# alanross/AlvaAR

Measured on AMD Instinct MI355X. Metric: frames/sec @640x480 2000kp; local-BA residuals/sec (20KFx3k pts), higher is better.
Workload: dtype u8/i16 image stages, f32 KLT, f64 pose+BA; 1 GPU; configs[1]: 640x480 RGBA stream, ~2000 keypoints/frame (cell 12), System::findCameraPose dataflow (fb-KLT -> P3P-LMedS -> PnP; keyframes: detect + describe, triangulate, map matching, local BA) via alva_system_find_camera_pose_device, steady state, frames resident in HBM; parallelism=1 independent camera streams, one per GPU, no collective on the data path

## Files before the change

### alvaar_amd/csrc/ba.hip

```cpp
#include "common.hpp"
#include "lm_device.hpp"
#include "wave_utils.hpp"
#include <chrono>
#include <cstdlib>
#include <algorithm>
#include <cmath>
#include <numeric>

namespace {

typedef double double4_t __attribute__((ext_vector_type(4)));

struct BaDev {
    int nKf, nPt, nObs, inv, dp, nc, n6, NP;
    int npd;
    int kpad;
    double K[4], huber_a;
    const int *obsKf;
    const double *obsUv;
    const int *ptPtr;
    const int *ancKf;
    const double *ancUv;
    const int *cidx;
    double *rowcol;
    const int *kfOf;
    const int *pairPerm;
    const int *pairPtr;
    double *Jobs;
    double *rs;
    double *chi2;
    uint8_t *depth;
    double *ptCost;
    double *Hpp;
    double *gp;
    double *Wt;
    double *M;
    double *Hcc;
    double *gc;
    double *sc, *sp, *dc, *dpd;
    double *hinv;
    double *Zt;
    double *Gpart;
    double *S;
    double *yc;
    double *yp;
    double *scal;
    double *h_scal;
    long long seq;
    double *partial;
    unsigned long long *dbg;
};
#define SOLVE_STAMP(k) do { if (B.dbg && threadIdx.x == 0) B.dbg[3072 + (k)] = wall_clock64(); } while (0)
#define ASM_STAMP(k) do { if (B.dbg && threadIdx.x == 0) B.dbg[3072 + 48 + (k)] = wall_clock64(); } while (0)

constexpr int KSPLIT = 8;

__device__ __forceinline__ double wave_sum(double v) {
#pragma unroll
    for (int off = 32; off > 0; off >>= 1) v += __shfl_down(v, off);
    return __shfl(v, 0);
}

template<bool INV, bool WANT_J>
__device__ __forceinline__ void point_body(const BaDev &B, const double *__restrict__ poses, const double *__restrict__ pts, const int BX_, const int BY_) {
    const int lane = threadIdx.x & 63;
    const int p = BX_ * 4 + (threadIdx.x >> 6);
    if (p >= B.nPt) return;
    constexpr int DP = INV ? 1 : 3;
    const int o0 = B.ptPtr[p], o1 = B.ptPtr[p + 1];
    double X[3], dJl[3] = {0, 0, 0};
    int a = -1;
    if (INV) {
        a = B.ancKf[p];
        Se3 Ta;
        se3_from_pose7(poses + 7 * a, Ta);
        const double zanch = 1.0 / pts[p];
        const double ap[3] = {zanch * ((B.ancUv[2 * p] - B.K[2]) / B.K[0]), zanch * ((B.ancUv[2 * p + 1] - B.K[3]) / B.K[1]), zanch};
        double Ra[3];
        for (int i = 0; i < 3; i++) Ra[i] = Ta.R[3 * i] * ap[0] + Ta.R[3 * i + 1] * ap[1] + Ta.R[3 * i + 2] * ap[2];
        for (int i = 0; i < 3; i++) {
            X[i] = Ra[i] + Ta.t[i];
            dJl[i] = -zanch * Ra[i];
        }
    } else {
        for (int i = 0; i < 3; i++) X[i] = pts[3 * p + i];
    }
    double cost = 0, hpp[DP * DP], gpv[DP], wanc[6 * DP];
#pragma unroll
    for (int i = 0; i < DP * DP; i++) hpp[i] = 0;
#pragma unroll
    for (int i = 0; i < DP; i++) gpv[i] = 0;
#pragma unroll
    for (int i = 0; i < 6 * DP; i++) wanc[i] = 0;
    for (int o = o0 + lane; o < o1; o += 64) {
        const int k = B.obsKf[o];
        Se3 T;
        se3_from_pose7(poses + 7 * k, T);
        double r[2], JR[6], chi2;
        int dpz;
        reproj<WANT_J>(T, B.K, X, B.obsUv[2 * o], B.obsUv[2 * o + 1], r, JR, chi2, dpz);
        B.chi2[o] = chi2;
        B.depth[o] = (uint8_t) dpz;
        double rho0, rho1;
        huber_rho(chi2, B.huber_a, 1, rho0, rho1);
        cost += 0.5 * rho0;
        if (WANT_J) {
            const double s = sqrt(rho1);
            double JH[6], Jo[12], Je[2 * DP];
// ... 57 lines not shown
                    const double w = wave_sum(wanc[i]);
                    if (lane == 0) B.Wt[(size_t) p * B.NP + 6 * ca + i] = w;
                }
            }
        }
    }
}
template<bool INV, bool WANT_J>
__global__ void __launch_bounds__(256) k_point(BaDev B, const double *__restrict__ poses, const double *__restrict__ pts) {
    point_body<INV, WANT_J>(B, poses, pts, blockIdx.x, blockIdx.y);
}

__device__ __forceinline__ void pairs_body(const BaDev &B, const int BX_, const int BY_) {
    const int lane = threadIdx.x & 63, wave = threadIdx.x >> 6;
    const int key = BX_;
    __shared__ double s_part[4][28];
    double v[32];
#pragma unroll
    for (int i = 0; i < 32; i++) v[i] = 0;
    for (int q = B.pairPtr[key] + threadIdx.x; q < B.pairPtr[key + 1]; q += 256) {
        const int o = B.pairPerm[q];
        double J[12];
#pragma unroll
        for (int i = 0; i < 12; i++) J[i] = B.Jobs[(size_t) o * 12 + i];
        const double r0 = B.rs[2 * (size_t) o], r1 = B.rs[2 * (size_t) o + 1];
        int t = 0;
#pragma unroll
        for (int x = 0; x < 6; x++) {
            v[21 + x] += J[x] * r0 + J[6 + x] * r1;
#pragma unroll
            for (int y = x; y < 6; y++) v[t++] += J[x] * J[y] + J[6 + x] * J[6 + y];
        }
    }
    wave_reduce_scatter32(v);
    if (!(lane & 1) && (lane >> 1) < 27) s_part[wave][lane >> 1] = v[0];
    __syncthreads();
    if (threadIdx.x < 27) B.M[(size_t) key * 27 + threadIdx.x] = ((s_part[0][threadIdx.x] + s_part[1][threadIdx.x]) + s_part[2][threadIdx.x]) + s_part[3][threadIdx.x];
}
__global__ void __launch_bounds__(256) k_pairs(BaDev B) {
    pairs_body(B, blockIdx.x, blockIdx.y);
}

__device__ __forceinline__ int tri6(int x, int y) {
    if (x > y) {
        const int t = x;
        x = y;
        y = t;
    }
    return x * 6 - x * (x - 1) / 2 + (y - x);
}

constexpr int ASM_NT = 1024;
static inline size_t assemble_lds(int n_kf) { return (size_t) 2 * n_kf * 27 * sizeof(double); }
__device__ __forceinline__ void assemble_body(const BaDev &B, int first) {
    extern __shared__ double s_rc[];
    __shared__ double s_red[5][ASM_NT / 64];
    __shared__ int s_kfof[64];
    const int nKf = B.nKf, n6 = B.n6, tid = threadIdx.x;
    ASM_STAMP(0);
    if (tid < B.nc && tid < 64) s_kfof[tid] = B.kfOf[tid];
    double *rowsum = s_rc, *colsum = s_rc + (size_t) nKf * 27;
    for (int e = tid; e < 2 * nKf * 27; e += ASM_NT) {
        const bool col = e >= nKf * 27;
        const int q = col ? e - nKf * 27 : e, k = q / 27, t = q - 27 * k;
        const size_t stride = col ? (size_t) nKf * 27 : 27, first_e = col ? (size_t) k * 27 + t : (size_t) k * nKf * 27 + t;
        double acc = 0;
        for (int j0 = 0; j0 < nKf; j0 += 8) {
            double v[8];
#pragma unroll
            for (int u = 0; u < 8; u++) v[u] = j0 + u < nKf ? B.M[first_e + (size_t) (j0 + u) * stride] : 0.0;
#pragma unroll
            for (int u = 0; u < 8; u++)
                if (j0 + u < nKf) acc += v[u];
        }
        s_rc[e] = acc;
    }
    __syncthreads();
    ASM_STAMP(1);
    double gm = 0;
    {
        const double *__restrict__ M = B.M;
        const int lane = tid & 63, wave = tid >> 6, NW = ASM_NT / 64;
        const bool lds_map = B.nc <= 64;
        for (int r0 = wave; r0 < n6; r0 += 2 * NW) {
            for (int c0 = lane; c0 < n6; c0 += 128) {
                double v[4];
                int er[4], ec[4];
#pragma unroll
                for (int u = 0; u < 4; u++) {
                    const int r = r0 + (u >> 1) * NW, c = c0 + (u & 1) * 64;
                    er[u] = r; ec[u] = c;
                    v[u] = 0;
                    if (r < n6 && c < n6) {
                        const int cr = r / 6, cc = c / 6, x = r - 6 * cr, y = c - 6 * cc;
                        const int kr = lds_map ? s_kfof[cr] : B.kfOf[cr], kc = lds_map ? s_kfof[cc] : B.kfOf[cc];
                        const int t = tri6(x, y);
                        if (B.inv) {
                            if (kr == kc) v[u] = rowsum[kr * 27 + t] + colsum[kr * 27 + t];
                            else v[u] = -(M[(size_t) (kr * nKf + kc) * 27 + t] + M[(size_t) (kc * nKf + kr) * 27 + t]);
                        } else {
                            if (kr == kc) v[u] = M[(size_t) (kr * nKf + kr) * 27 + t];
                        }
                    }
                }
#pragma unroll
                for (int u = 0; u < 4; u++)
                    if (er[u] < n6 && ec[u] < n6) {
                        B.Hcc[(size_t) er[u] * n6 + ec[u]] = v[u];
                        if (first && er[u] == ec[u]) B.sc[er[u]] = 1.0 / (1.0 + sqrt(v[u]));
                    }
            }
        }
        for (int r = tid; r < n6; r += ASM_NT) {
            const int cr = r / 6, x = r - 6 * cr, kr = lds_map ? s_kfof[cr] : B.kfOf[cr];
            const double g = B.inv ? rowsum[kr * 27 + 21 + x] - colsum[kr * 27 + 21 + x] : M[(size_t) (kr * nKf + kr) * 27 + 21 + x];
            B.gc[r] = g;
            gm = fmax(gm, fabs(g));
        }
    }
    ASM_STAMP(2);
    if (first)
        for (int i = tid; i < B.npd; i += ASM_NT) {
            const int p = i / B.dp, x = i % B.dp;
            B.sp[i] = 1.0 / (1.0 + sqrt(B.Hpp[(size_t) p * B.dp * B.dp + x * B.dp + x]));
        }
    double cost = 0, mcc = 0, sn = 0, xn = 0;
    for (int i = tid; i < B.npd; i += ASM_NT) gm = fmax(gm, fabs(B.gp[i]));
    for (int p = tid; p < B.nPt; p += ASM_NT) {
        cost += B.ptCost[p];
        mcc += B.partial[3 * (size_t) p];
        sn += B.partial[3 * (size_t) p + 1];
        xn += B.partial[3 * (size_t) p + 2];
    }
    const int lane = tid & 63, wave = tid >> 6;
#pragma unroll
    for (int off = 32; off > 0; off >>= 1) {
        gm = fmax(gm, __shfl_xor(gm, off));
        cost += __shfl_xor(cost, off);
        mcc += __shfl_xor(mcc, off);
        sn += __shfl_xor(sn, off);
        xn += __shfl_xor(xn, off);
    }
    if (lane == 0) {
        s_red[0][wave] = gm; s_red[1][wave] = cost; s_red[2][wave] = mcc; s_red[3][wave] = sn; s_red[4][wave] = xn;
    }
    __syncthreads();
    ASM_STAMP(3);
    if (tid == 0) {
        double g2 = 0, c2 = 0, m2 = 0, s2 = 0, x2 = 0;
        for (int w = 0; w < ASM_NT / 64; w++) {
            g2 = fmax(g2, s_red[0][w]);
            c2 += s_red[1][w]; m2 += s_red[2][w]; s2 += s_red[3][w]; x2 += s_red[4][w];
        }
        const double *cam = B.partial + 3 * (size_t) B.nPt;
        B.scal[0] = c2;
        B.scal[3] = g2;
        B.scal[1] = m2 + cam[0];
        B.scal[2] = s2 + cam[1];
        B.scal[4] = x2 + cam[2];
        if (B.h_scal) {
            B.h_scal[0] = c2; B.h_scal[1] = m2 + cam[0]; B.h_scal[2] = s2 + cam[1]; B.h_scal[3] = g2;
            B.h_scal[4] = x2 + cam[2]; B.h_scal[5] = B.scal[5]; B.h_scal[6] = B.scal[6]; B.h_scal[7] = B.scal[7];
            __threadfence_system();
            __hip_atomic_store(reinterpret_cast<long long *>(B.h_scal + 8), B.seq, __ATOMIC_RELEASE, __HIP_MEMORY_SCOPE_SYSTEM);
        }
    }
}
__global__ void __launch_bounds__(ASM_NT) k_assemble(BaDev B, int first) { assemble_body(B, first); }

template<int DP>
__device__ __forceinline__ void prep_body(const BaDev &B, double radius, int refresh, const int BX_, const int BY_) {
    const int lane = threadIdx.x & 63;
    const int p = BX_ * 4 + (threadIdx.x >> 6);
    if (p >= B.nPt) return;
    double Mx[DP * DP], Hi[DP * DP], L[DP * DP], gs[DP], dpd[DP];
#pragma unroll
    for (int x = 0; x < DP; x++) {
        const int i = p * DP + x;
        if (refresh) {
            dpd[x] = fmin(fmax(B.Hpp[(size_t) p * DP * DP + x * DP + x] * B.sp[i] * B.sp[i], 1e-6), 1e32);
            if (lane == 0) B.dpd[i] = dpd[x];
        } else {
            dpd[x] = B.dpd[i];
        }
    }
#pragma unroll
    for (int x = 0; x < DP; x++) {
        gs[x] = B.gp[(size_t) p * DP + x] * B.sp[p * DP + x];
#pragma unroll
        for (int y = 0; y < DP; y++)
            Mx[x * DP + y] = B.Hpp[(size_t) p * DP * DP + x * DP + y] * B.sp[p * DP + x] * B.sp[p * DP + y] + (x == y ? dpd[x] / radius : 0.0);
    }
    if (DP == 1) {
        Hi[0] = 1.0 / Mx[0];
        L[0] = sqrt(Hi[0]);
    } else {
        for (int c = 0; c < DP; c++) {
            double A3[DP * DP], e[DP];
            for (int i = 0; i < DP * DP; i++) A3[i] = Mx[i];
            for (int i = 0; i < DP; i++) e[i] = (i == c);
            chol_solve_dense(A3, e, DP);
            for (int i = 0; i < DP; i++) Hi[i * DP + c] = e[i];
        }
        for (int i = 0; i < DP * DP; i++) L[i] = 0;
        for (int j = 0; j < DP; j++) {
            double d = Hi[j * DP + j];
            for (int k = 0; k < j; k++) d -= L[j * DP + k] * L[j * DP + k];
            d = sqrt(d);
            L[j * DP + j] = d;
            for (int i = j + 1; i < DP; i++) {
                double s = Hi[i * DP + j];
                for (int k = 0; k < j; k++) s -= L[i * DP + k] * L[j * DP + k];
                L[i * DP + j] = s / d;
            }
        }
    }
    if (lane == 0)
        for (int i = 0; i < DP * DP; i++) B.hinv[(size_t) p * DP * DP + i] = Hi[i];
    for (int r = lane; r < B.NP; r += 64) {
#pragma unroll
        for (int y = 0; y < DP; y++) {
            double v = 0;
            if (r < B.n6) {
#pragma unroll
                for (int x = 0; x < DP; x++) v += B.sc[r] * B.Wt[((size_t) p * DP + x) * B.NP + r] * B.sp[p * DP + x] * L[x * DP + y];
            } else if (r == B.n6) {
#pragma unroll
                for (int x = 0; x < DP; x++) v += L[x * DP + y] * gs[x];
            }
            B.Zt[((size_t) p * DP + y) * B.NP + r] = v;
        }
    }
}
template<int DP>
__global__ void __launch_bounds__(256) k_prep(BaDev B, double radius, int refresh) {
    prep_body<DP>(B, radius, refresh, blockIdx.x, blockIdx.y);
}

__device__ __forceinline__ void gemm_body(const BaDev &B, const int BX_, const int BY_) {
    const int tiles = B.NP / 16;
    const int ti = BX_ / tiles, tj = BX_ % tiles, ks = BY_;
    const int lane = threadIdx.x;
    const int chunk = B.kpad / KSPLIT;
    const int k0 = ks * chunk;
    double4_t acc = {0, 0, 0, 0};
    const double *Za = B.Zt + (size_t) (k0 + (lane >> 4)) * B.NP + ti * 16 + (lane & 15);
    const double *Zb = B.Zt + (size_t) (k0 + (lane >> 4)) * B.NP + tj * 16 + (lane & 15);
    int k = 0;
    for (; k + 32 <= chunk; k += 32) {
        double a[8], b[8];
#pragma unroll
        for (int u = 0; u < 8; u++) {
            a[u] = Za[(size_t) (k + 4 * u) * B.NP];
            b[u] = Zb[(size_t) (k + 4 * u) * B.NP];
        }
#pragma unroll
        for (int u = 0; u < 8; u++) acc = __builtin_amdgcn_mfma_f64_16x16x4f64(a[u], b[u], acc, 0, 0, 0);
    }
    for (; k < chunk; k += 4) {
        const double a = Za[(size_t) k * B.NP], b = Zb[(size_t) k * B.NP];
        acc = __builtin_amdgcn_mfma_f64_16x16x4f64(a, b, acc, 0, 0, 0);
    }
    double *G = B.Gpart + ((size_t) ks * B.NP + ti * 16) * B.NP + tj * 16;
#pragma unroll
    for (int r = 0; r < 4; r++) G[(size_t) ((lane >> 4) + 4 * r) * B.NP + (lane & 15)] = acc[r];
}
__global__ void __launch_bounds__(64) k_gemm(BaDev B) {
    gemm_body(B, blockIdx.x, blockIdx.y);
}

#ifndef ALVA_SOLVE_LOOKAHEAD
#define ALVA_SOLVE_LOOKAHEAD 1
#endif
constexpr int SOLVE_NT = 256, NB = 16;

__device__ __forceinline__ void reduced_system_body(const BaDev &B, double radius, int refresh, const int BX_, const int BY_) {
    const int n = B.n6, np = (n + NB - 1) / NB * NB, ld = np + 1;
    const int e = BX_ * 256 + threadIdx.x;
    if (e < np * np) {
        const int r = e / np, c = e - r * np;
        double v = r == c ? 1.0 : 0.0;
        if (r < n && c < n) {
            double g = 0;
#pragma unroll
            for (int ks = 0; ks < KSPLIT; ks++) g += B.Gpart[((size_t) ks * B.NP + r) * B.NP + c];
            const double h = B.Hcc[(size_t) r * n + c] * B.sc[r] * B.sc[c];
            v = h - g;
            if (r == c) {
                double dcr = B.dc[r];
                if (refresh) {
                    dcr = fmin(fmax(h, 1e-6), 1e32);
                    B.dc[r] = dcr;
                }
                v += dcr / radius;
            }
        }
        B.S[(size_t) r * ld + c] = v;
    } else if (e < np * np + np) {
        const int r = e - np * np;
        double v = 0;
        if (r < n) {
            double g = 0;
#pragma unroll
            for (int ks = 0; ks < KSPLIT; ks++) g += B.Gpart[((size_t) ks * B.NP + r) * B.NP + n];
            v = B.gc[r] * B.sc[r] - g;
        }
        B.S[(size_t) np * ld + r] = v;
    }
}
__global__ void __launch_bounds__(256) k_reduced_system(BaDev B, double radius, int refresh) {
    reduced_system_body(B, radius, refresh, blockIdx.x, blockIdx.y);
}

template<bool IN_LDS>
__device__ __forceinline__ void solve_body(const BaDev &B, double radius, const int BX_, const int BY_) {
    extern __shared__ double s_S[];
    const int n = B.n6, np = (n + NB - 1) / NB * NB, ld = np + 1, nb = np / NB;
    __shared__ double s_z[NB];
    __shared__ int s_ok;
    SOLVE_STAMP(0);
    double *S = IN_LDS ? s_S : B.S;
    double *y = IN_LDS ? s_S + (size_t) np * ld : B.S + (size_t) np * ld;
    constexpr int TILE_LUT = 1024;
    __shared__ unsigned short s_tile[TILE_LUT];
    auto fill_lut = [&]() {
        for (int t = threadIdx.x; t < TILE_LUT; t += SOLVE_NT) {
            int ta = (int) ((sqrtf(8.f * (float) t + 1.f) - 1.f) * 0.5f);
            while (ta * (ta + 1) / 2 > t) ta--;
            while ((ta + 1) * (ta + 2) / 2 <= t) ta++;
            s_tile[t] = (unsigned short) ((ta << 8) | (t - ta * (ta + 1) / 2));
        }
    };
    if (IN_LDS) {
        const int total = np * ld + np;
        bool lut_done = false;
        for (int e0 = threadIdx.x; e0 < total || !lut_done; e0 += 32 * SOLVE_NT) {
            double v[32];
#pragma unroll
            for (int u = 0; u < 32; u++) {
                const int e = e0 + u * SOLVE_NT;
                v[u] = e < total ? B.S[e] : 0.0;
            }
            if (!lut_done) {
                fill_lut();
                lut_done = true;
            }
#pragma unroll
            for (int u = 0; u < 32; u++) {
                const int e = e0 + u * SOLVE_NT;
                if (e < total) s_S[e] = v[u];
            }
        }
    } else {
        fill_lut();
    }
    if (threadIdx.x == 0) s_ok = 1;
    __syncthreads();
    SOLVE_STAMP(1);
    const int lane = threadIdx.x & 63;
    auto diag_factor = [&](const int base) {
// ... 441 lines not shown
        L.gmax = scal[3];
        L.last = L.cur;
    } else {
        const int cand = 1 - L.cur;
        L.last = cand;
        const double cand_cost = scal[0], mcc = scal[1], step_norm = sqrt(scal[2]);
        const bool okstep = scal[5] != 0.0 && isfinite(mcc);
        if (!okstep || !(mcc > 0)) {
            if (++L.invalid >= 5) {
                L.ok = 0;
                stop = true;
            } else {
                lm.rejected();
                L.nsummaries++;
            }
        } else {
            L.invalid = 0;
            if (step_norm <= 1e-8 * (L.x_norm + 1e-8)) stop = true;
            else if (fabs(L.x_cost - cand_cost) <= L.function_tolerance * L.x_cost) stop = true;
            else {
                const double rel = (L.x_cost - cand_cost) / mcc;
                if (rel > 1e-3) {
                    L.cur = cand;
                    L.x_cost = cand_cost;
                    L.gmax = scal[3];
                    L.x_norm = sqrt(scal[4]);
                    lm.accepted(rel);
                    L.nsucc++;
                } else {
                    lm.rejected();
                }
                L.nsummaries++;
            }
        }
    }
    L.radius = lm.radius; L.decrease_factor = lm.decrease_factor; L.reuse_diagonal = lm.reuse_diagonal;
    if (stop || L.iteration >= L.max_iters || L.gmax <= 1e-10 || L.radius <= 1e-32) {
        L.step = 0;
        return;
    }
    L.iteration++;
    L.diag = L.reuse_diagonal ? 0 : 1;
    L.reuse_diagonal = 1;
    L.step = 1;
}

#define LM_EVAL_SEL(first)                                  \
    if (!(first) && !L->step) return;                       \
    const int set = (first) ? L->cur : 1 - L->cur;          \
    const BaDev &B = dB[set];
template<bool INV>
__global__ void __launch_bounds__(256) k_point_lm(const BaDev *__restrict__ dB, const BaLmDev *__restrict__ L, int first) {
    LM_EVAL_SEL(first)
    point_body<INV, true>(B, L->P[set], L->T[set], blockIdx.x, 0);
}
__global__ void __launch_bounds__(256) k_pairs_lm(const BaDev *__restrict__ dB, const BaLmDev *__restrict__ L, int first) {
    LM_EVAL_SEL(first)
    pairs_body(B, blockIdx.x, 0);
}
__global__ void __launch_bounds__(ASM_NT) k_assemble_lm(const BaDev *__restrict__ dB, BaLmDev *L, int first) {
    LM_EVAL_SEL(first)
    assemble_body(B, first);
    if (threadIdx.x == 0) {
        BaLmDev S = *L;
        lm_after_eval(S, B.scal, first);
        S.evals++;
        *L = S;
        double *h = S.h_pub + ((S.evals & 1) ? 16 : 0);
        h[0] = S.step; h[1] = S.iteration; h[2] = S.nsummaries; h[3] = S.initial; h[4] = S.x_cost; h[5] = S.nsucc; h[6] = S.ok;
        h[7] = (double) (S.cur | (S.last << 8));
        __threadfence_system();
        __hip_atomic_store(reinterpret_cast<long long *>(S.h_pub + 8), S.evals, __ATOMIC_RELEASE, __HIP_MEMORY_SCOPE_SYSTEM);
    }
}
template<int DP>
__global__ void __launch_bounds__(256) k_prep_lm(const BaDev *__restrict__ dB, const BaLmDev *__restrict__ L) {
    if (!L->step) return;
    prep_body<DP>(dB[L->cur], L->radius, L->diag, blockIdx.x, 0);
}
__global__ void __launch_bounds__(64) k_gemm_lm(const BaDev *__restrict__ dB, const BaLmDev *__restrict__ L) {
    if (!L->step) return;
    gemm_body(dB[L->cur], blockIdx.x, blockIdx.y);
}
__global__ void __launch_bounds__(256) k_reduced_system_lm(const BaDev *__restrict__ dB, const BaLmDev *__restrict__ L) {
    if (!L->step) return;
    reduced_system_body(dB[L->cur], L->radius, L->diag, blockIdx.x, 0);
}
template<bool IN_LDS>
__global__ void __launch_bounds__(SOLVE_NT) k_solve_lm(const BaDev *__restrict__ dB, const BaLmDev *__restrict__ L) {
    if (!L->step) return;
    solve_body<IN_LDS>(dB[L->cur], L->radius, 0, 0);
}
template<int DP>
__global__ void __launch_bounds__(256) k_backsub_lm(const BaDev *__restrict__ dB, const BaLmDev *__restrict__ L) {
    if (!L->step) return;
    const int c = L->cur;
    backsub_body<DP>(dB[c], L->radius, L->T[c], L->T[1 - c], L->P[c], L->P[1 - c], blockIdx.x, 0);
}
struct BaIn {
    int n_kf;
    double *h_poses;
    const uint8_t *h_kf_const;
    const double *h_calib;
    int inv_depth, n_pt;
    const int *h_pt_anchor_kf;
    const double *h_pt_anchor_uv;
    double *h_pt_param;
    int n_obs;
    const int *h_obs_kf, *h_obs_pt;
    const double *h_obs_uv;
    double huber_chi2;
};

struct BaCsr {
    const int *h_pt_ptr;
    double chi2_threshold;
    unsigned long long *h_bad_bits;
    int *h_n_bad;
};

struct BaHost {
    BaDev B{};
    std::vector<int> cidx, order;
    bool grouped_ = false;
    bool csr_ = false;
    int *d_pairKey = nullptr, *d_pairHist = nullptr;
    unsigned long long *d_badBits = nullptr;
    int n_chunks = 0;
    int *d_obsKf = nullptr, *d_ptPtr = nullptr, *d_ancKf = nullptr, *d_cidx = nullptr, *d_pairPerm = nullptr, *d_pairPtr = nullptr, *d_kfOf = nullptr;
    double *d_obsUv = nullptr, *d_ancUv = nullptr, *d_xp = nullptr, *d_cp = nullptr, *d_xt = nullptr, *d_ct = nullptr;
    size_t in_bytes = 0, bytes = 0;
    size_t np16 = 0, solve_lds = 0;
    LmState lm;
    double x_cost = 0, gmax = 0, x_norm = -1, initial = 0;
    int iteration = 0, nsucc = 1, invalid = 0, nsummaries = 1, ok = 1;
    bool need_restore = false, done = false;
    double *xp = nullptr, *xt = nullptr, *cp = nullptr, *ct = nullptr;
    BaLmDev *d_lm = nullptr;
    BaDev *d_desc = nullptr;
// ... 25 lines not shown
        bytes = layout(nullptr);
        return ALVA_OK;
    }
    size_t layout(uint8_t *base) {
        const size_t nObs = (size_t) B.nObs, nPt = (size_t) B.nPt, npd = (size_t) B.npd, n6 = (size_t) B.n6, NP = (size_t) B.NP, dp = (size_t) B.dp;
        const size_t n_kf = (size_t) B.nKf;
        uint8_t *cur = base;
        d_obsKf = carve<int>(cur, nObs);
        d_obsUv = carve<double>(cur, nObs * 2);
        d_ptPtr = carve<int>(cur, nPt + 1);
        d_ancKf = carve<int>(cur, nPt);
        d_ancUv = carve<double>(cur, nPt * 2);
        d_cidx = carve<int>(cur, n_kf);
        d_kfOf = carve<int>(cur, n_kf);
        if (!csr_) {
            d_pairPerm = carve<int>(cur, nObs);
            d_pairPtr = carve<int>(cur, n_kf * n_kf + 1);
        }
        d_xp = carve<double>(cur, n_kf * 7);
        d_xt = carve<double>(cur, npd);
        d_lm = carve<BaLmDev>(cur, 1);
        d_desc = carve<BaDev>(cur, 2);
        in_bytes = (size_t) (cur - base);
        if (csr_) {
            d_pairPerm = carve<int>(cur, nObs);
            d_pairPtr = carve<int>(cur, n_kf * n_kf + 1);
            d_pairKey = carve<int>(cur, nObs);
            d_pairHist = carve<int>(cur, (size_t) n_chunks * n_kf * n_kf);
            d_badBits = carve<unsigned long long>(cur, nObs / 64 + 2);
        }
        B.chi2 = carve<double>(cur, nObs);
        B.depth = carve<uint8_t>(cur, nObs);
        B.Jobs = carve<double>(cur, nObs * 12);
        B.rs = carve<double>(cur, nObs * 2);
        B.ptCost = carve<double>(cur, nPt);
        B.Hpp = carve<double>(cur, npd * dp);
        B.gp = carve<double>(cur, npd);
        B.Wt = carve<double>(cur, npd * NP);
        B.Zt = carve<double>(cur, (size_t) B.kpad * NP);
        B.M = carve<double>(cur, n_kf * n_kf * 27);
        B.rowcol = carve<double>(cur, n_kf * 27 * 2);
        B.Hcc = carve<double>(cur, n6 * n6);
        B.gc = carve<double>(cur, n6);
        B.sc = carve<double>(cur, n6);
        B.sp = carve<double>(cur, npd);
        B.dc = carve<double>(cur, n6);
        B.dpd = carve<double>(cur, npd);
        B.hinv = carve<double>(cur, npd * dp);
        B.Gpart = carve<double>(cur, (size_t) KSPLIT * NP * NP);
        B.S = carve<double>(cur, (n6 + 16) * (n6 + 17) + n6 + 16);
        B.yc = carve<double>(cur, NP);
        B.yp = carve<double>(cur, npd);
        B.scal = carve<double>(cur, 64);
        B.dbg = alva_kstamp_buffer();
        B.partial = carve<double>(cur, nPt * 3 + 8);
        d_cp = carve<double>(cur, n_kf * 7);
        d_ct = carve<double>(cur, npd);
        B2.chi2 = carve<double>(cur, nObs);
        B2.depth = carve<uint8_t>(cur, nObs);
        B2.Jobs = carve<double>(cur, nObs * 12);
        B2.rs = carve<double>(cur, nObs * 2);
        B2.ptCost = carve<double>(cur, nPt);
        B2.Hpp = carve<double>(cur, npd * dp);
        B2.gp = carve<double>(cur, npd);
        B2.Wt = carve<double>(cur, npd * NP);
        B2.M = carve<double>(cur, n_kf * n_kf * 27);
        B2.Hcc = carve<double>(cur, n6 * n6);
        B2.gc = carve<double>(cur, n6);
        return (size_t) (cur - base);
    }
    int build(const BaIn &in, uint8_t *base, uint8_t *stage) {
        const int n_kf = in.n_kf, n_pt = in.n_pt, n_obs = in.n_obs;
        const size_t nPt = (size_t) n_pt, npd = (size_t) B.npd;
        layout(stage);
        int *h_obsKf = d_obsKf, *h_ptPtr = d_ptPtr, *h_ancKf = d_ancKf, *h_cidx = d_cidx, *h_kfOf = d_kfOf, *h_pairPerm = d_pairPerm, *h_pairPtr = d_pairPtr;
        double *h_obsUv = d_obsUv, *h_ancUv = d_ancUv, *h_xp = d_xp, *h_xt = d_xt;
        layout(base);
        B.obsKf = d_obsKf; B.obsUv = d_obsUv; B.ptPtr = d_ptPtr; B.ancKf = d_ancKf; B.ancUv = d_ancUv; B.cidx = d_cidx; B.kfOf = d_kfOf;
        B.pairPerm = d_pairPerm; B.pairPtr = d_pairPtr;
        order.resize((size_t) n_obs);
        static thread_local std::vector<int> pairKey, cursor;
        pairKey.resize((size_t) n_obs);
        for (size_t p2 = 0; p2 <= nPt; p2++) h_ptPtr[p2] = 0;
        const size_t nPairs = (size_t) n_kf * n_kf;
        for (size_t i = 0; i <= nPairs; i++) h_pairPtr[i] = 0;
        bool grouped = true;
        for (int o = 1; o < n_obs && grouped; o++) grouped = in.h_obs_pt[o] >= in.h_obs_pt[o - 1];
        grouped_ = grouped;
        if (grouped) {
            for (int o = 0; o < n_obs; o++) order[(size_t) o] = o;
        } else {
            cursor.assign((size_t) n_pt + 1, 0);
            for (int o = 0; o < n_obs; o++) cursor[(size_t) in.h_obs_pt[o] + 1]++;
            for (int p2 = 0; p2 < n_pt; p2++) cursor[(size_t) p2 + 1] += cursor[(size_t) p2];
            for (int o = 0; o < n_obs; o++) order[(size_t) cursor[(size_t) in.h_obs_pt[o]]++] = o;
        }
        for (int q = 0; q < n_obs; q++) {
            const int o = order[(size_t) q], pt = in.h_obs_pt[o], kf = in.h_obs_kf[o];
            h_obsKf[q] = kf;
            h_obsUv[2 * (size_t) q] = in.h_obs_uv[2 * o];
            h_obsUv[2 * (size_t) q + 1] = in.h_obs_uv[2 * o + 1];
            h_ptPtr[(size_t) pt + 1]++;
            const int anc = in.inv_depth ? in.h_pt_anchor_kf[pt] : kf;
            ALVA_ARG(anc >= 0 && anc < n_kf);
            const int key = kf * n_kf + anc;
            pairKey[(size_t) q] = key;
// ... 127 lines not shown
        for (int k = 0; k < in.n_kf; k++)
            if (cidx[(size_t) k] >= 0) memcpy(in.h_poses + 7 * k, r_poses + 7 * (size_t) k, 56);
        if (grouped_) {
            if (h_chi2) memcpy(h_chi2, chi2s, (size_t) in.n_obs * 8);
            if (h_depth_pos) memcpy(h_depth_pos, deps, (size_t) in.n_obs);
        } else {
            for (int q = 0; q < in.n_obs; q++) {
                if (h_chi2) h_chi2[order[(size_t) q]] = chi2s[(size_t) q];
                if (h_depth_pos) h_depth_pos[order[(size_t) q]] = deps[(size_t) q];
            }
        }
        if (h_info) {
            h_info[0] = nsummaries;
            h_info[1] = initial;
            h_info[2] = x_cost;
            h_info[3] = nsucc;
        }
    }
    size_t chi_bytes() const { return (size_t) ((uint8_t *) B.depth - (uint8_t *) B.chi2) + (size_t) B.nObs; }
};

}

static int ba_drive(alva_ctx *ctx, const BaIn &in, const BaCsr *csr, int max_iters, double function_tolerance, double *h_chi2,
                    uint8_t *h_depth_pos, double *h_info, int *h_ok) {
    const int n_kf = in.n_kf, n_pt = in.n_pt, n_obs = in.n_obs, inv_depth = in.inv_depth;
    *h_ok = 1;
    if (h_info) memset(h_info, 0, 4 * sizeof(double));
    const auto t_begin = std::chrono::steady_clock::now();
    BaHost H;
    int rc = H.sizes(in, csr);
    if (rc) return rc;
    BaDev &B = H.B;
    const int dp = B.dp;
    const size_t nObs = (size_t) n_obs, npd = (size_t) B.npd, NP = (size_t) B.NP;
    uint8_t *base = nullptr;
    rc = alva_ctx_scratch(ctx, 4, H.bytes, (void **) &base);
    if (rc) return rc;
    const size_t res_bytes = (nObs * 9 + 511) / 256 * 256 + (size_t) n_kf * 56 + 256 + npd * 8 + 256;
    uint8_t *pin = nullptr;
    rc = alva_ctx_pinned(ctx, 256 + std::max(H.in_bytes, res_bytes), (void **) &pin);
    if (rc) return rc;
    uint8_t *stage = pin + 256;
    hipStream_t st = ctx->stream;
    const auto t_sized = std::chrono::steady_clock::now();
    ALVA_HIP(alva_stream_sync(st));
    const auto t_synced = std::chrono::steady_clock::now();
    rc = csr ? H.build_csr(in, *csr, base, stage) : H.build(in, base, stage);
    if (rc) return rc;
    const auto t_built = std::chrono::steady_clock::now();
    H.stage_lm(base, stage, max_iters, function_tolerance, reinterpret_cast<double *>(pin));
    ALVA_HIP(hipMemcpyAsync(base, stage, H.in_bytes, hipMemcpyHostToDevice, st));
    if (csr) H.enqueue_pairs(st);
    ALVA_HIP(hipMemsetAsync(B.Wt, 0, (size_t) ((uint8_t *) B.Zt - (uint8_t *) B.Wt) + (size_t) B.kpad * NP * 8, st));
    const auto t_up = std::chrono::steady_clock::now();

    const dim3 gPt((unsigned) alva_divup(std::max(n_pt, 1), 4)), blk(256);
    static const bool poll = alva_poll_enabled();
    double *pin_scal = reinterpret_cast<double *>(pin);
    long long eval_seq = 0;
    reinterpret_cast<volatile long long *>(pin_scal + 8)[0] = 0;
    B.h_scal = poll ? pin_scal : nullptr;
    const size_t np16 = H.np16, solve_lds = H.solve_lds;
    const bool solve_in_lds = solve_lds <= 152 * 1024;
    if (solve_in_lds && solve_lds > 48 * 1024)
        ALVA_HIP(hipFuncSetAttribute(reinterpret_cast<const void *>(k_solve<true>), hipFuncAttributeMaxDynamicSharedMemorySize, 152 * 1024));
    auto eval = [&](const double *xp, const double *xt, bool first) -> int {
        if (n_pt > 0) {
            if (inv_depth) hipLaunchKernelGGL((k_point<true, true>), gPt, blk, 0, st, B, xp, xt);
            else hipLaunchKernelGGL((k_point<false, true>), gPt, blk, 0, st, B, xp, xt);
        }
        hipLaunchKernelGGL(k_pairs, dim3((unsigned) (n_kf * n_kf)), blk, 0, st, B);
        B.seq = ++eval_seq;
        hipLaunchKernelGGL(k_assemble, dim3(1), dim3(ASM_NT), assemble_lds(n_kf), st, B, first ? 1 : 0);
        ALVA_LAUNCH_CHECK();
        return ALVA_OK;
    };
    double scal[8];
    auto read_scal = [&]() -> int {
        if (poll) {
            const volatile long long *flag = reinterpret_cast<const volatile long long *>(pin_scal + 8);
            if (!alva_wait_until([&] { return *flag == eval_seq; }, st)) {
                alva_set_error("local BA: evaluation %lld never published its scalars", eval_seq);
                return ALVA_ERR_STATE;
            }
            memcpy(scal, pin_scal, sizeof(scal));
            return ALVA_OK;
        }
        ALVA_HIP(hipMemcpyAsync(pin_scal, B.scal, sizeof(scal), hipMemcpyDeviceToHost, st));
        ALVA_HIP(alva_stream_sync(st));
        memcpy(scal, pin_scal, sizeof(scal));
        return ALVA_OK;
    };

    int last_set = 0, cur_set = 0;
    if (poll) {
        ALVA_HIP(hipMemsetAsync(H.B2.Wt, 0, (size_t) B.npd * NP * 8, st));
        const BaDev *dB = H.d_desc;
        BaLmDev *dL = H.d_lm;
        const int tiles = B.NP / 16, np16i = (int) np16;
        const dim3 gBs(n_pt > 0 ? gPt.x + 1 : 1);
        auto eval_lm = [&](int first) {
            if (n_pt > 0) {
                if (inv_depth) hipLaunchKernelGGL(k_point_lm<true>, gPt, blk, 0, st, dB, (const BaLmDev *) dL, first);
                else hipLaunchKernelGGL(k_point_lm<false>, gPt, blk, 0, st, dB, (const BaLmDev *) dL, first);
            }
            hipLaunchKernelGGL(k_pairs_lm, dim3((unsigned) (n_kf * n_kf)), blk, 0, st, dB, (const BaLmDev *) dL, first);
            hipLaunchKernelGGL(k_assemble_lm, dim3(1), dim3(ASM_NT), assemble_lds(n_kf), st, dB, dL, first);
        };
        auto step_lm = [&]() {
            if (n_pt > 0) {
                if (dp == 1) hipLaunchKernelGGL(k_prep_lm<1>, gPt, blk, 0, st, dB, (const BaLmDev *) dL);
                else hipLaunchKernelGGL(k_prep_lm<3>, gPt, blk, 0, st, dB, (const BaLmDev *) dL);
            }
            hipLaunchKernelGGL(k_gemm_lm, dim3((unsigned) (tiles * tiles), KSPLIT), dim3(64), 0, st, dB, (const BaLmDev *) dL);
            if (np16 > 0)
                hipLaunchKernelGGL(k_reduced_system_lm, dim3((unsigned) alva_divup(np16i * np16i + np16i, 256)), blk, 0, st, dB, (const BaLmDev *) dL);
            if (solve_in_lds) hipLaunchKernelGGL(k_solve_lm<true>, dim3(1), dim3(SOLVE_NT), solve_lds, st, dB, (const BaLmDev *) dL);
            else hipLaunchKernelGGL(k_solve_lm<false>, dim3(1), dim3(SOLVE_NT), 0, st, dB, (const BaLmDev *) dL);
            if (dp == 1) hipLaunchKernelGGL(k_backsub_lm<1>, gBs, blk, 0, st, dB, (const BaLmDev *) dL);
            else hipLaunchKernelGGL(k_backsub_lm<3>, gBs, blk, 0, st, dB, (const BaLmDev *) dL);
            eval_lm(0);
        };
        if (solve_in_lds && solve_lds > 48 * 1024)
            ALVA_HIP(hipFuncSetAttribute(reinterpret_cast<const void *>(k_solve_lm<true>), hipFuncAttributeMaxDynamicSharedMemorySize, 152 * 1024));
        eval_lm(1);
        int issued = 0;
        if (max_iters > 0) {
            step_lm();
            issued = 1;
        }
        ALVA_LAUNCH_CHECK();
        long long seen = 0;
        double pub[8];
        for (;;) {
            const volatile long long *flag = reinterpret_cast<const volatile long long *>(pin_scal + 8);
            long long f = 0;
            if (!alva_wait_until([&] { return (f = *flag) >= seen + 1; }, st)) {
                alva_set_error("local BA: publication %lld of the device minimiser never came", seen + 1);
                return ALVA_ERR_STATE;
            }
            memcpy(pub, pin_scal + ((f & 1) ? 16 : 0), sizeof(pub));
            seen = f;
            if (pub[0] == 0.0) break;
            if (issued < max_iters) {
                step_lm();
                issued++;
                ALVA_LAUNCH_CHECK();
            } else if (seen >= (long long) max_iters + 1) {
                break;
            }
        }
        H.nsummaries = (int) pub[2]; H.initial = pub[3]; H.x_cost = pub[4]; H.nsucc = (int) pub[5]; H.ok = (int) pub[6];
        cur_set = ((int) pub[7]) & 0xff;
        last_set = ((int) pub[7]) >> 8;
    } else {
    rc = eval(H.d_xp, H.d_xt, true);
    if (rc) return rc;
    rc = read_scal();
    if (rc) return rc;
    H.x_cost = H.initial = scal[0];
    H.gmax = scal[3];
    LmState &lm = H.lm;
    while (true) {
        if (H.loop_ends(max_iters)) break;
        H.iteration++;
        if (H.need_restore) {
            rc = eval(H.xp, H.xt, false);
            if (rc) return rc;
            H.need_restore = false;
// ... 310 lines not shown
```

Baseline: 4098 frames/s.

## Parallelize BA assembly across workgroups and fuse reduced-system build into GEMM

The single-workgroup assemble kernel in the LM path becomes a multi-workgroup row-parallel assemble. The last-arriving workgroup, found with an atomic counter, computes the global scalars. The separate reduced-system kernel is folded into the split-K GEMM, where the last K-slice block for each tile sums the partials and writes S. Host memsets of Wt and Zt padding move into the first-eval kernels. This removes kernel launches and a serial single-block stage, at the cost of atomic last-block synchronisation and relaxed-store/fence ordering that must be correct.

```diff
diff --git a/alvaar_amd/csrc/ba.hip b/alvaar_amd/csrc/ba.hip
--- a/alvaar_amd/csrc/ba.hip
+++ b/alvaar_amd/csrc/ba.hip
@@ -49,11 +49,15 @@
     long long seq;
     double *partial;
     unsigned long long *dbg;
+    int *sync;
 };
 #define SOLVE_STAMP(k) do { if (B.dbg && threadIdx.x == 0) B.dbg[3072 + (k)] = wall_clock64(); } while (0)
 #define ASM_STAMP(k) do { if (B.dbg && threadIdx.x == 0) B.dbg[3072 + 48 + (k)] = wall_clock64(); } while (0)
 
 constexpr int KSPLIT = 8;
+
+__device__ __forceinline__ void st_wt(double *p, double v) { __hip_atomic_store(p, v, __ATOMIC_RELAXED, __HIP_MEMORY_SCOPE_AGENT); }
+__device__ __forceinline__ void vm_drain() { asm volatile("s_waitcnt vmcnt(0)" ::: "memory"); }
 
 __device__ __forceinline__ double wave_sum(double v) {
 #pragma unroll
@@ -217,9 +221,9 @@
 
 constexpr int ASM_NT = 1024;
 static inline size_t assemble_lds(int n_kf) { return (size_t) 2 * n_kf * 27 * sizeof(double); }
+__device__ __forceinline__ void assemble_scalars(const BaDev &B, int first, double gm);
 __device__ __forceinline__ void assemble_body(const BaDev &B, int first) {
     extern __shared__ double s_rc[];
-    __shared__ double s_red[5][ASM_NT / 64];
     __shared__ int s_kfof[64];
     const int nKf = B.nKf, n6 = B.n6, tid = threadIdx.x;
     ASM_STAMP(0);
@@ -283,6 +287,13 @@
             gm = fmax(gm, fabs(g));
         }
     }
+    assemble_scalars(B, first, gm);
+}
+__global__ void __launch_bounds__(ASM_NT) k_assemble(BaDev B, int first) { assemble_body(B, first); }
+
+__device__ __forceinline__ void assemble_scalars(const BaDev &B, int first, double gm) {
+    __shared__ double s_red[5][ASM_NT / 64];
+    const int tid = threadIdx.x;
     ASM_STAMP(2);
     if (first)
         for (int i = tid; i < B.npd; i += ASM_NT) {
@@ -331,7 +342,68 @@
         }
     }
 }
-__global__ void __launch_bounds__(ASM_NT) k_assemble(BaDev B, int first) { assemble_body(B, first); }
+
+constexpr int ASM_MAX_WG = 64;
+__device__ __forceinline__ bool assemble_rows_body(const BaDev &B, int first) {
+    __shared__ double s_rc1[2 * 27];
+    __shared__ int s_kfof[ASM_MAX_WG];
+    __shared__ int s_last;
+    const int nKf = B.nKf, n6 = B.n6, nc = B.nc, tid = threadIdx.x;
+    const double *__restrict__ M = B.M;
+    const bool lds_map = nc <= ASM_MAX_WG;
+    if (lds_map && tid < nc) s_kfof[tid] = B.kfOf[tid];
+    for (int cr = blockIdx.x; cr < nc; cr += gridDim.x) {
+        const int kr = B.kfOf[cr];
+        if (tid < 2 * 27) {
+            const bool col = tid >= 27;
+            const int t = col ? tid - 27 : tid;
+            const size_t stride = col ? (size_t) nKf * 27 : 27, first_e = col ? (size_t) kr * 27 + t : (size_t) kr * nKf * 27 + t;
+            double acc = 0;
+            for (int j0 = 0; j0 < nKf; j0 += 8) {
+                double v[8];
+#pragma unroll
+                for (int u = 0; u < 8; u++) v[u] = j0 + u < nKf ? M[first_e + (size_t) (j0 + u) * stride] : 0.0;
+#pragma unroll
+                for (int u = 0; u < 8; u++)
+                    if (j0 + u < nKf) acc += v[u];
+            }
+            s_rc1[tid] = acc;
+        }
+        __syncthreads();
+        for (int e = tid; e < 6 * n6; e += ASM_NT) {
+            const int x = e / n6, c = e - x * n6, r = 6 * cr + x;
+            const int cc = c / 6, y = c - 6 * cc;
+            const int kc = lds_map ? s_kfof[cc] : B.kfOf[cc];
+            const int t = tri6(x, y);
+            double v = 0;
+            if (B.inv) {
+                if (kr == kc) v = s_rc1[t] + s_rc1[27 + t];
+                else v = -(M[(size_t) (kr * nKf + kc) * 27 + t] + M[(size_t) (kc * nKf + kr) * 27 + t]);
+            } else {
+                if (kr == kc) v = M[(size_t) (kr * nKf + kr) * 27 + t];
+            }
+            st_wt(B.Hcc + (size_t) r * n6 + c, v);
+            if (first && r == c) st_wt(B.sc + r, 1.0 / (1.0 + sqrt(v)));
+        }
+        if (tid < 6) st_wt(B.gc + 6 * cr + tid, B.inv ? s_rc1[21 + tid] - s_rc1[27 + 21 + tid] : M[(size_t) (kr * nKf + kr) * 27 + 21 + tid]);
+        __syncthreads();
+    }
+    vm_drain();
+    __syncthreads();
+    if (tid == 0) s_last = __hip_atomic_fetch_add(B.sync, 1, __ATOMIC_RELAXED, __HIP_MEMORY_SCOPE_AGENT) == (int) gridDim.x - 1;
+    __syncthreads();
+    if (!s_last) return false;
+    if (tid == 0) {
+        __builtin_amdgcn_fence(__ATOMIC_ACQUIRE, "agent");
+        vm_drain();
+        __hip_atomic_store(B.sync, 0, __ATOMIC_RELAXED, __HIP_MEMORY_SCOPE_AGENT);
+    }
+    __syncthreads();
+    double gm = 0;
+    for (int r = tid; r < n6; r += ASM_NT) gm = fmax(gm, fabs(B.gc[r]));
+    assemble_scalars(B, first, gm);
+    return true;
+}
 
 template<int DP>
 __device__ __forceinline__ void prep_body(const BaDev &B, double radius, int refresh, const int BX_, const int BY_) {
@@ -402,6 +474,7 @@
     prep_body<DP>(B, radius, refresh, blockIdx.x, blockIdx.y);
 }
 
+template<bool WT = false>
 __device__ __forceinline__ void gemm_body(const BaDev &B, const int BX_, const int BY_) {
     const int tiles = B.NP / 16;
     const int ti = BX_ / tiles, tj = BX_ % tiles, ks = BY_;
@@ -428,7 +501,10 @@
     }
     double *G = B.Gpart + ((size_t) ks * B.NP + ti * 16) * B.NP + tj * 16;
 #pragma unroll
-    for (int r = 0; r < 4; r++) G[(size_t) ((lane >> 4) + 4 * r) * B.NP + (lane & 15)] = acc[r];
+    for (int r = 0; r < 4; r++) {
+        if (WT) st_wt(G + (size_t) ((lane >> 4) + 4 * r) * B.NP + (lane & 15), acc[r]);
+        else G[(size_t) ((lane >> 4) + 4 * r) * B.NP + (lane & 15)] = acc[r];
+    }
 }
 __global__ void __launch_bounds__(64) k_gemm(BaDev B) {
     gemm_body(B, blockIdx.x, blockIdx.y);
@@ -439,38 +515,46 @@
 #endif
 constexpr int SOLVE_NT = 256, NB = 16;
 
+__device__ __forceinline__ double reduced_elem(const BaDev &B, double radius, int refresh, const int r, const int c) {
+    const int n = B.n6;
+    double v = r == c ? 1.0 : 0.0;
+    if (r < n && c < n) {
+        double g = 0;
+#pragma unroll
+        for (int ks = 0; ks < KSPLIT; ks++) g += B.Gpart[((size_t) ks * B.NP + r) * B.NP + c];
+        const double h = B.Hcc[(size_t) r * n + c] * B.sc[r] * B.sc[c];
+        v = h - g;
+        if (r == c) {
+            double dcr = B.dc[r];
+            if (refresh) {
+                dcr = fmin(fmax(h, 1e-6), 1e32);
+                B.dc[r] = dcr;
+            }
+            v += dcr / radius;
+        }
+    }
+    return v;
+}
+__device__ __forceinline__ double reduced_rhs(const BaDev &B, const int r) {
+    const int n = B.n6;
+    double v = 0;
+    if (r < n) {
+        double g = 0;
+#pragma unroll
+        for (int ks = 0; ks < KSPLIT; ks++) g += B.Gpart[((size_t) ks * B.NP + r) * B.NP + n];
+        v = B.gc[r] * B.sc[r] - g;
+    }
+    return v;
+}
 __device__ __forceinline__ void reduced_system_body(const BaDev &B, double radius, int refresh, const int BX_, const int BY_) {
     const int n = B.n6, np = (n + NB - 1) / NB * NB, ld = np + 1;
     const int e = BX_ * 256 + threadIdx.x;
     if (e < np * np) {
         const int r = e / np, c = e - r * np;
-        double v = r == c ? 1.0 : 0.0;
-        if (r < n && c < n) {
-            double g = 0;
-#pragma unroll
-            for (int ks = 0; ks < KSPLIT; ks++) g += B.Gpart[((size_t) ks * B.NP + r) * B.NP + c];
-            const double h = B.Hcc[(size_t) r * n + c] * B.sc[r] * B.sc[c];
-            v = h - g;
-            if (r == c) {
-                double dcr = B.dc[r];
-                if (refresh) {
-                    dcr = fmin(fmax(h, 1e-6), 1e32);
-                    B.dc[r] = dcr;
-                }
-                v += dcr / radius;
-            }
-        }
-        B.S[(size_t) r * ld + c] = v;
+        B.S[(size_t) r * ld + c] = reduced_elem(B, radius, refresh, r, c);
     } else if (e < np * np + np) {
         const int r = e - np * np;
-        double v = 0;
-        if (r < n) {
-            double g = 0;
-#pragma unroll
-            for (int ks = 0; ks < KSPLIT; ks++) g += B.Gpart[((size_t) ks * B.NP + r) * B.NP + n];
-            v = B.gc[r] * B.sc[r] - g;
-        }
-        B.S[(size_t) np * ld + r] = v;
+        B.S[(size_t) np * ld + r] = reduced_rhs(B, r);
     }
 }
 __global__ void __launch_bounds__(256) k_reduced_system(BaDev B, double radius, int refresh) {
@@ -1018,15 +1102,33 @@
 template<bool INV>
 __global__ void __launch_bounds__(256) k_point_lm(const BaDev *__restrict__ dB, const BaLmDev *__restrict__ L, int first) {
     LM_EVAL_SEL(first)
+    if (first) {
+        constexpr int DP = INV ? 1 : 3;
+        const int p = blockIdx.x * 4 + (threadIdx.x >> 6);
+        if (p < B.nPt) {
+            for (int s = 0; s < 2; s++) {
+                double *w = dB[s].Wt + (size_t) p * DP * B.NP;
+                for (int i = threadIdx.x & 63; i < DP * B.NP; i += 64) w[i] = 0.0;
+            }
+            vm_drain();
+        }
+    }
     point_body<INV, true>(B, L->P[set], L->T[set], blockIdx.x, 0);
 }
 __global__ void __launch_bounds__(256) k_pairs_lm(const BaDev *__restrict__ dB, const BaLmDev *__restrict__ L, int first) {
     LM_EVAL_SEL(first)
+    if (first) {
+        const int tiles = B.NP / 16, stride = (int) gridDim.x * 256, t0 = (int) blockIdx.x * 256 + (int) threadIdx.x;
+        for (int i = t0; i < 1 + tiles * tiles; i += stride) B.sync[i] = 0;
+        double *zpad = B.Zt + (size_t) B.npd * B.NP;
+        const size_t npad = (size_t) (B.kpad - B.npd) * B.NP;
+        for (size_t i = (size_t) t0; i < npad; i += (size_t) stride) zpad[i] = 0.0;
+    }
     pairs_body(B, blockIdx.x, 0);
 }
 __global__ void __launch_bounds__(ASM_NT) k_assemble_lm(const BaDev *__restrict__ dB, BaLmDev *L, int first) {
     LM_EVAL_SEL(first)
-    assemble_body(B, first);
+    if (!assemble_rows_body(B, first)) return;
     if (threadIdx.x == 0) {
         BaLmDev S = *L;
         lm_after_eval(S, B.scal, first);
@@ -1046,11 +1148,30 @@
 }
 __global__ void __launch_bounds__(64) k_gemm_lm(const BaDev *__restrict__ dB, const BaLmDev *__restrict__ L) {
     if (!L->step) return;
-    gemm_body(dB[L->cur], blockIdx.x, blockIdx.y);
-}
-__global__ void __launch_bounds__(256) k_reduced_system_lm(const BaDev *__restrict__ dB, const BaLmDev *__restrict__ L) {
-    if (!L->step) return;
-    reduced_system_body(dB[L->cur], L->radius, L->diag, blockIdx.x, 0);
+    const BaDev &B = dB[L->cur];
+    gemm_body<true>(B, blockIdx.x, blockIdx.y);
+    vm_drain();
+    int last = 0;
+    if (threadIdx.x == 0) last = __hip_atomic_fetch_add(B.sync + 1 + blockIdx.x, 1, __ATOMIC_RELAXED, __HIP_MEMORY_SCOPE_AGENT) == KSPLIT - 1;
+    if (!__shfl(last, 0)) return;
+    if (threadIdx.x == 0) {
+        __builtin_amdgcn_fence(__ATOMIC_ACQUIRE, "agent");
+        vm_drain();
+        __hip_atomic_store(B.sync + 1 + blockIdx.x, 0, __ATOMIC_RELAXED, __HIP_MEMORY_SCOPE_AGENT);
+    }
+    __syncthreads();
+    const int tiles = B.NP / 16, ti = blockIdx.x / tiles, tj = blockIdx.x % tiles;
+    const int n = B.n6, np = (n + NB - 1) / NB * NB, ld = np + 1;
+    const double radius = L->radius;
+    const int refresh = L->diag;
+    for (int e = threadIdx.x; e < 256; e += 64) {
+        const int r = ti * 16 + (e >> 4), c = tj * 16 + (e & 15);
+        if (r < np && c < np) B.S[(size_t) r * ld + c] = reduced_elem(B, radius, refresh, r, c);
+    }
+    if (tj == n / 16 && threadIdx.x < 16) {
+        const int r = ti * 16 + threadIdx.x;
+        if (r < np) B.S[(size_t) np * ld + r] = reduced_rhs(B, r);
+    }
 }
 template<bool IN_LDS>
 __global__ void __launch_bounds__(SOLVE_NT) k_solve_lm(const BaDev *__restrict__ dB, const BaLmDev *__restrict__ L) {
@@ -1182,6 +1303,7 @@
         B.yc = carve<double>(cur, NP);
         B.yp = carve<double>(cur, npd);
         B.scal = carve<double>(cur, 64);
+        B.sync = carve<int>(cur, 1 + (NP / 16) * (NP / 16));
         B.dbg = alva_kstamp_buffer();
         B.partial = carve<double>(cur, nPt * 3 + 8);
         d_cp = carve<double>(cur, n_kf * 7);
@@ -1415,11 +1537,11 @@
     H.stage_lm(base, stage, max_iters, function_tolerance, reinterpret_cast<double *>(pin));
     ALVA_HIP(hipMemcpyAsync(base, stage, H.in_bytes, hipMemcpyHostToDevice, st));
     if (csr) H.enqueue_pairs(st);
-    ALVA_HIP(hipMemsetAsync(B.Wt, 0, (size_t) ((uint8_t *) B.Zt - (uint8_t *) B.Wt) + (size_t) B.kpad * NP * 8, st));
+    static const bool poll = alva_poll_enabled();
+    if (!poll) ALVA_HIP(hipMemsetAsync(B.Wt, 0, (size_t) ((uint8_t *) B.Zt - (uint8_t *) B.Wt) + (size_t) B.kpad * NP * 8, st));
     const auto t_up = std::chrono::steady_clock::now();
 
     const dim3 gPt((unsigned) alva_divup(std::max(n_pt, 1), 4)), blk(256);
-    static const bool poll = alva_poll_enabled();
     double *pin_scal = reinterpret_cast<double *>(pin);
     long long eval_seq = 0;
     reinterpret_cast<volatile long long *>(pin_scal + 8)[0] = 0;
@@ -1458,18 +1580,18 @@
 
     int last_set = 0, cur_set = 0;
     if (poll) {
-        ALVA_HIP(hipMemsetAsync(H.B2.Wt, 0, (size_t) B.npd * NP * 8, st));
         const BaDev *dB = H.d_desc;
         BaLmDev *dL = H.d_lm;
-        const int tiles = B.NP / 16, np16i = (int) np16;
+        const int tiles = B.NP / 16;
         const dim3 gBs(n_pt > 0 ? gPt.x + 1 : 1);
+        const dim3 gAsm((unsigned) std::max(1, std::min(B.nc, ASM_MAX_WG)));
         auto eval_lm = [&](int first) {
             if (n_pt > 0) {
                 if (inv_depth) hipLaunchKernelGGL(k_point_lm<true>, gPt, blk, 0, st, dB, (const BaLmDev *) dL, first);
                 else hipLaunchKernelGGL(k_point_lm<false>, gPt, blk, 0, st, dB, (const BaLmDev *) dL, first);
             }
             hipLaunchKernelGGL(k_pairs_lm, dim3((unsigned) (n_kf * n_kf)), blk, 0, st, dB, (const BaLmDev *) dL, first);
-            hipLaunchKernelGGL(k_assemble_lm, dim3(1), dim3(ASM_NT), assemble_lds(n_kf), st, dB, dL, first);
+            hipLaunchKernelGGL(k_assemble_lm, gAsm, dim3(ASM_NT), 0, st, dB, dL, first);
         };
         auto step_lm = [&]() {
             if (n_pt > 0) {
@@ -1477,8 +1599,6 @@
                 else hipLaunchKernelGGL(k_prep_lm<3>, gPt, blk, 0, st, dB, (const BaLmDev *) dL);
             }
             hipLaunchKernelGGL(k_gemm_lm, dim3((unsigned) (tiles * tiles), KSPLIT), dim3(64), 0, st, dB, (const BaLmDev *) dL);
-            if (np16 > 0)
-                hipLaunchKernelGGL(k_reduced_system_lm, dim3((unsigned) alva_divup(np16i * np16i + np16i, 256)), blk, 0, st, dB, (const BaLmDev *) dL);
             if (solve_in_lds) hipLaunchKernelGGL(k_solve_lm<true>, dim3(1), dim3(SOLVE_NT), solve_lds, st, dB, (const BaLmDev *) dL);
             else hipLaunchKernelGGL(k_solve_lm<false>, dim3(1), dim3(SOLVE_NT), 0, st, dB, (const BaLmDev *) dL);
             if (dp == 1) hipLaunchKernelGGL(k_backsub_lm<1>, gBs, blk, 0, st, dB, (const BaLmDev *) dL);
```

Result: slower. 3991 frames/s (-2.6%).
